# raulmur/ORB_SLAM

Measured on AMD Instinct MI355X. Metric: frames/s ORB extract+match @640x480, 1000 kp, higher is better.
Workload: dtype u8; 1 GPU; vga: 640x480 grayscale stream, 8 levels, nFeatures 1000, S-blocks frames, extract + Hamming top-2 match vs previous frame (BASELINE.json configs[1] + the frame-to-frame match of the metric); resident_frames_per_gpu=2048, lanes=4, parity_checked_frames=0, parity_mismatches=0, library_build_id=b66c8a98a159e636, lane_placement=2

## Files before the change

include/orbx.h:

```cpp
#ifndef ORBX_H
#define ORBX_H

#include <stddef.h>
#include <stdint.h>

#ifdef __cplusplus
extern "C" {
#endif

#define ORBX_OK             0
#define ORBX_EMPTY          1
#define ORBX_ERR_ARG       -1
#define ORBX_ERR_DEVICE    -2
#define ORBX_ERR_CAPACITY  -3
#define ORBX_ERR_GEOMETRY  -4

#define ORBX_HARRIS_SCORE 0
#define ORBX_FAST_SCORE   1

#define ORBX_BLUR_X86_SSE2 0
#define ORBX_BLUR_HALF_UP  1

#define ORBX_FP_ISO          0
#define ORBX_FP_GCC_CONTRACT 1
// ... 109 lines not shown
int orbx_event_destroy(int device, void* event);
int orbx_event_record(void* event, void* stream);
int orbx_stream_wait_event(void* stream, void* event);
int orbx_device_copy_async(void* d_dst, const void* d_src, size_t bytes, void* stream);
int orbx_host_alloc(int device, size_t bytes, void** h_ptr);
int orbx_host_free(int device, void* h_ptr);
int orbx_device_upload_async(void* d_dst, const void* h_src, size_t bytes, void* stream);
int orbx_device_download_async(void* h_dst, const void* d_src, size_t bytes, void* stream);

int orbm_distinctive(const uint8_t* desc, const int32_t* seg_off, int npoints, int32_t* best_idx, int32_t* best_median, int device);
int orbm_distinctive_device(const uint8_t* d_desc, const int32_t* d_seg_off, int npoints, int32_t* d_best_idx,
                            int32_t* d_best_median, void* stream);

#define ORBX_DBG_PLANE      0
#define ORBX_DBG_BLUR       1
#define ORBX_DBG_NMS        2
#define ORBX_DBG_LEVEL_KPS  3
#define ORBX_DBG_BANDS      4
int orbx_debug_set_stop_after(orbx_extractor* h, int stage);
int orbx_debug_set_blur_on_demand(orbx_extractor* h, int mode);
int orbx_debug_stage_timing(orbx_extractor* h, int enable);
int orbx_debug_stage_time(orbx_extractor* h, int stage, double* total_ms, long* launches);
int orbx_debug_level_size(const orbx_extractor* h, int level, int* w, int* hgt);
long orbx_debug_fetch(orbx_extractor* h, int what, int frame, int level, void* host_out, long cap_bytes);
int orbx_debug_geometry(const orbx_params* p, int w, int hgt, int32_t* out, int cap_levels);
int orbx_debug_nth_element(const float* resp, int n, int nth, int32_t* out_perm, int device);
int orbx_debug_eval_math(int kind, const float* in0, const float* in1, float* out0, float* out1, int n, int device);
int orbx_debug_eval_compass(const uint32_t* c, const uint32_t* e, const uint32_t* w, const uint32_t* nn, const uint32_t* ss, uint32_t* out, int n, int t, int device);
int orbx_debug_eval_blur_window(const uint8_t* windows, uint8_t* out, int n, int rounding, int general, int device);

#ifdef __cplusplus
}
#endif
#endif
```

orb_slam_amd/capi.py:

```python
import ctypes
import os
import numpy as np

_HERE = os.path.dirname(os.path.abspath(__file__))
LIB_PATH = os.environ.get("ORBX_LIB") or os.path.join(_HERE, "liborbx.so")

ORBX_OK, ORBX_EMPTY = 0, 1
ORBX_ERR_ARG, ORBX_ERR_DEVICE, ORBX_ERR_CAPACITY, ORBX_ERR_GEOMETRY = -1, -2, -3, -4
HARRIS_SCORE, FAST_SCORE = 0, 1
BLUR_X86_SSE2, BLUR_HALF_UP = 0, 1
DBG_PLANE, DBG_BLUR, DBG_NMS, DBG_LEVEL_KPS, DBG_BANDS = 0, 1, 2, 3, 4
(ST_PYRAMID, ST_FAST_CELLS, ST_QUOTA, ST_CELL_SELECT, ST_LEVEL_SELECT, ST_BLUR, ST_DESCRIBE) = range(7)

KP_DTYPE = np.dtype([("x", "<f4"), ("y", "<f4"), ("size", "<f4"), ("angle", "<f4"),
                     ("response", "<f4"), ("octave", "<i4"), ("class_id", "<i4")])

EXPORTS = [
    "orbx_default_params", "orbx_create", "orbx_destroy", "orbx_get_levels", "orbx_get_scale_factor",
    "orbx_max_keypoints", "orbx_last_error", "orbx_build_id", "orbx_extract", "orbx_extract_batch_device", "orbx_extract_batch_device_phases", "orbx_extract_batch",
    "orbx_to_gray_device", "orbx_extract_color", "orbx_extract_batch_device_color", "orbx_extract_batch_color",
    "orbm_hamming256", "orbm_match_top2", "orbm_match_top2_device", "orbm_match_top2_batch_device", "orbm_match_top2_masked", "orbm_match_top2_masked_device",
    "orbm_count_accepted", "orbm_match_top2_segments", "orbm_match_top2_segments_device", "orbm_distinctive", "orbm_distinctive_device",
    "orbx_device_alloc", "orbx_device_free", "orbx_device_upload", "orbx_device_download",
    "orbx_stream_create", "orbx_stream_create_priority", "orbx_stream_destroy", "orbx_stream_synchronize", "orbx_event_create", "orbx_event_destroy", "orbx_event_record",
    "orbx_stream_wait_event", "orbx_device_copy_async", "orbx_host_alloc", "orbx_host_free", "orbx_device_upload_async", "orbx_device_download_async", "orbx_debug_set_stop_after", "orbx_debug_set_blur_on_demand", "orbx_debug_level_size", "orbx_debug_fetch",
    "orbx_debug_eval_math", "orbx_debug_eval_compass", "orbx_debug_eval_blur_window", "orbx_debug_stage_timing", "orbx_debug_stage_time", "orbx_debug_nth_element", "orbx_debug_geometry",
    "orbm_debug_set_match_path",
    "orbm_debug_get_match_path",
]
EXPORTS_F = [
    "orbf_image_bounds", "orbf_undistort_grid", "orbf_undistort_grid_batch_device", "orbf_features_in_area",
    "orbf_features_in_area_device",
]
EXPORTS_S = ["orbs_lds_bytes", "orbs_debug_set_buckets", "orbs_debug_set_wide_max", "orbs_three_maxima", "orbs_window_search_batch_device", "orbs_list_search_batch_device",
             "orbs_bow_ranges_batch_device", "orbs_triangulation_search_batch_device", "orbs_epipolar_bound", "orbs_agreement_batch_device",
             "orbs_bow_rows_search_batch_device", "orbs_bow_rows_search", "orbs_tri_rows_search_batch_device", "orbs_tri_rows_search"]
PHASE_PYRAMID, PHASE_DETECT, PHASE_DESCRIBE, PHASE_ALL = 1, 2, 4, 7
RULE_MAPPOINTS, RULE_WINDOW, RULE_BEST, RULE_INIT, RULE_BOW, RULE_FREE, RULE_TRIANGULATION = 0, 1, 2, 3, 4, 5, 6
TH_HIGH, TH_LOW = 100, 50
EXPORTS_V = [
    "orbv_create", "orbv_load_text", "orbv_destroy", "orbv_info", "orbv_descend", "orbv_descend_device",
    "orbv_transform", "orbv_transform_batch_device", "orbv_score",
]
EXPORTS_D = ["orbd_create", "orbd_destroy", "orbd_size", "orbd_add", "orbd_add_batch_device", "orbd_erase", "orbd_clear",
             "orbd_query_batch_device", "orbd_query"]
EXPORTS_P = ["orbp_create", "orbp_destroy", "orbp_capacity", "orbp_size", "orbp_clear", "orbp_put", "orbp_put_device", "orbp_erase", "orbp_get",
             "orbp_project_batch_device", "orbp_track_batch_device", "orbp_track", "orbp_project_source_batch_device",
             "orbp_track_source_batch_device", "orbp_track_source", "orbp_refresh_batch_device", "orbp_refresh", "orbp_fuse_batch_device",
# ... 161 lines not shown
        L.orbx_extract_batch_color.argtypes = [vp, vp, vp, ci, ci, ci, ci, ci, vp, vp, vp, ci, vp, vp]
        L.orbm_hamming256.argtypes = [vp, vp]
        L.orbm_match_top2.argtypes = [vp, ci, vp, ci, vp, vp, vp, ci]
        L.orbm_match_top2_device.argtypes = [vp, ci, vp, ci, vp, vp, vp, vp]
        L.orbm_match_top2_batch_device.argtypes = [vp, vp, vp, vp, ci, ci, vp, vp, vp, vp]
        L.orbm_match_top2_masked.argtypes = [vp, ci, vp, ci, vp, vp, vp, vp, ci]
        L.orbm_match_top2_masked_device.argtypes = [vp, ci, vp, ci, vp, vp, vp, vp, vp]
        L.orbm_count_accepted.argtypes = [vp, vp, ci, ci, cf]
        L.orbm_debug_set_match_path.argtypes = [ci]
        L.orbm_debug_get_match_path.argtypes = []
        L.orbs_debug_set_buckets.argtypes = [ci]
        L.orbs_debug_set_wide_max.argtypes = [ci]
        L.orbm_match_top2_segments.argtypes = [vp, ci, vp, ci, vp, vp, vp, vp, vp, ci]
        L.orbm_match_top2_segments_device.argtypes = [vp, ci, vp, ci, vp, vp, vp, vp, vp, vp]
        L.orbx_device_alloc.argtypes = [ci, ctypes.c_size_t, ctypes.POINTER(vp)]
        L.orbx_device_free.argtypes = [ci, vp]
        L.orbx_device_upload.argtypes = [ci, vp, vp, ctypes.c_size_t]
        L.orbx_device_download.argtypes = [ci, vp, vp, ctypes.c_size_t]
        L.orbm_distinctive.argtypes = [vp, vp, ci, vp, vp, ci]
        L.orbm_distinctive_device.argtypes = [vp, vp, ci, vp, vp, vp]
        L.orbx_debug_set_stop_after.argtypes = [vp, ci]
        L.orbx_debug_set_blur_on_demand.argtypes = [vp, ci]
        L.orbx_debug_level_size.argtypes = [vp, ci, ctypes.POINTER(ci), ctypes.POINTER(ci)]
        L.orbx_debug_fetch.argtypes = [vp, ci, ci, ci, vp, cl]
        L.orbx_debug_fetch.restype = cl
        L.orbx_debug_eval_math.argtypes = [ci, vp, vp, vp, vp, ci, ci]
        L.orbx_debug_eval_compass.argtypes = [vp, vp, vp, vp, vp, vp, ci, ci, ci]
        L.orbx_debug_eval_blur_window.argtypes = [vp, vp, ci, ci, ci, ci]
        L.orbx_debug_nth_element.argtypes = [vp, ci, ci, vp, ci]
        L.orbx_debug_geometry.argtypes = [ctypes.POINTER(Params), ci, ci, vp, ci]
        L.orbx_debug_stage_timing.argtypes = [vp, ci]
        L.orbx_debug_stage_time.argtypes = [vp, ci, ctypes.POINTER(ctypes.c_double), ctypes.POINTER(cl)]
        L.orbf_image_bounds.argtypes = [ctypes.POINTER(Camera), ctypes.POINTER(Bounds)]
        L.orbf_undistort_grid.argtypes = [ctypes.POINTER(Camera), ctypes.POINTER(Bounds), vp, ci, vp, vp, vp, ci]
        L.orbf_undistort_grid_batch_device.argtypes = [ctypes.POINTER(Camera), ctypes.POINTER(Bounds), vp, vp, ci, ci, vp, vp, vp, vp]
        L.orbf_features_in_area.argtypes = [ctypes.POINTER(Bounds), vp, ci, vp, vp, vp, vp, ci, vp, vp, ci, ci]
        L.orbf_features_in_area_device.argtypes = [ctypes.POINTER(Bounds), vp, ci, vp, vp, vp, vp, ci, vp, vp, ci, vp, vp]
        L.orbs_lds_bytes.argtypes = [ci, ci]
        L.orbs_lds_bytes.restype = ctypes.c_size_t
        L.orbs_three_maxima.argtypes = [vp, ci, vp]
        L.orbs_three_maxima.restype = None
        L.orbs_window_search_batch_device.argtypes = [ctypes.POINTER(Bounds), ctypes.POINTER(SearchParams), vp, vp, vp, vp, vp, ci, vp,
                                                      vp, vp, vp, vp, vp, vp, ci, ci, vp, vp, vp, vp, vp, vp]
        L.orbs_list_search_batch_device.argtypes = [ctypes.POINTER(SearchParams), vp, vp, vp, vp, vp, ci, vp, vp, vp, vp, vp, vp, vp, ci, ci,
                                                    vp, vp, vp, vp, vp, vp]
        L.orbs_bow_ranges_batch_device.argtypes = [vp, vp, vp, vp, vp, vp, ci, ci, vp, vp, vp]
# ... 291 lines not shown
        if rc != ORBX_OK:
            raise OrbxError(rc, "orbx_debug_set_blur_on_demand")

    STAGE_NAMES = ["pyramid", "fast_cells", "quota", "cell_select", "level_select", "blur", "describe"]

    def stage_timing(self, enable):
        self.L.orbx_debug_stage_timing(self.h, enable)

    def stage_times(self):
        res = {}
        for i, name in enumerate(self.STAGE_NAMES):
            ms, n = ctypes.c_double(), ctypes.c_long()
            self.L.orbx_debug_stage_time(self.h, i, ctypes.byref(ms), ctypes.byref(n))
            res[name] = (ms.value, n.value)
        return res

    def level_size(self, level):
        w, hh = ctypes.c_int(), ctypes.c_int()
        rc = self.L.orbx_debug_level_size(self.h, level, ctypes.byref(w), ctypes.byref(hh))
        if rc != ORBX_OK:
            raise self._err(rc)
        return w.value, hh.value

    def fetch_plane(self, what, level, frame=0):
        w, hh = self.level_size(level)
        out = np.empty((hh, w), dtype=np.uint8)
        rc = self.L.orbx_debug_fetch(self.h, what, frame, level, out.ctypes.data, out.nbytes)
        if rc < 0:
            raise self._err(rc)
        return out

    def fetch_bands(self, level, frame=0):
        out = np.zeros((16384, 8), dtype=np.int32)
        rc = self.L.orbx_debug_fetch(self.h, DBG_BANDS, frame, level, out.ctypes.data, out.nbytes)
        if rc < 0:
            raise self._err(rc)
        return out[:rc // 32].copy()

    def fetch_level_keypoints(self, level, frame=0):
        out = np.zeros((4 * self.max_keypoints + 64, 3), dtype=np.int32)
        rc = self.L.orbx_debug_fetch(self.h, DBG_LEVEL_KPS, frame, level, out.ctypes.data, out.nbytes)
        if rc < 0:
            raise self._err(rc)
        n = rc // 12
        xy = out[:n, :2].copy()
        resp = out[:n, 2].copy().view(np.float32)
# ... 992 lines not shown
```

orb_slam_amd/csrc/k_pyramid.hip:

```cpp
#include <algorithm>
#include <type_traits>

#include "orbx_device.h"
#include "orbx_launch.h"

namespace orbx {


template <bool ALIGNED, bool WINDOW, bool GATHER>
__device__ __forceinline__ void k_resize_body(Batch b, int level) {
    extern __shared__ __attribute__((aligned(16))) uint8_t s_src[];
    const DevGeom& g = b.g;
    const LevelGeom& L = g.lv[level];
    const int RZ_SRC_W = L.rz_pitch;
    const LevelGeom& P = g.lv[level - 1];
    const int tiles_x = (L.w + 255) / 256, tiles_y = (L.h + RZ_ROWS - 1) / RZ_ROWS;
    int frame, tile;
    if (!frame_item(b, blockIdx.x, tiles_x * tiles_y, frame, tile)) return;
    const int tile_y = tile / tiles_x, tile_x = tile - tile_y * tiles_x;
    const int tid = threadIdx.x, lane = tid & 63, wave = wave_id();
    const int bx0 = tile_x * 256, by0 = tile_y * RZ_ROWS;
    const int bx1 = min(bx0 + 255, L.w - 1), by1 = min(by0 + RZ_ROWS - 1, L.h - 1);
    long long sstride;
    const uint8_t* src = plain_plane<GATHER>(b, P, level - 1, frame, sstride);
    const ResizeX* tx = b.tabx + L.tabx_off;
// ... 96 lines not shown
        }
        return;
    }
#pragma unroll
    for (int j = 0; j < RZ_ROWS / 4; j++) {
        const int dy = by0 + wave + 4 * j;
        if (dy >= L.h) break;
        const ResizeY ry = ty[dy];
        const uint8_t* q0 = s_src + (ry.sy0 - r0) * RZ_SRC_W - c0;
        const uint8_t* q1 = s_src + (ry.sy1 - r0) * RZ_SRC_W - c0;
        uint32_t packed = 0;
#pragma unroll
        for (int k = 0; k < 4; k++) {
            const int px = resize_px(q0[rx[k].sx], q0[rx[k].sx1], q1[rx[k].sx], q1[rx[k].sx1], rx[k].a0, rx[k].a1, ry.b0, ry.b1);
            packed |= (uint32_t)(px & 255) << (8 * k);
        }
        *reinterpret_cast<uint32_t*>(dplane + (long long)dy * L.stride + dx0) = packed;
    }
}
template <bool ALIGNED, bool WINDOW>
__global__ __launch_bounds__(256) void k_resize(Batch b, int level) { k_resize_body<ALIGNED, WINDOW, false>(b, level); }
template <bool ALIGNED, bool WINDOW>
__global__ __launch_bounds__(256) void k_resize_gather(Batch b, int level) { k_resize_body<ALIGNED, WINDOW, true>(b, level); }

template <bool ALIGNED, bool GATHER>
__global__ __launch_bounds__(256) void k_pyramid(Batch b, int group) {
    extern __shared__ __attribute__((aligned(16))) uint8_t s_lv[];
    const DevGeom& g = b.g;
    const PyrGroup& pg = g.pyr[group];
    const int frame = blockIdx.z, ix = blockIdx.x, iy = blockIdx.y;
    const int tid = threadIdx.x;
    const int l0 = pg.l0, depth = pg.depth;
    if (group == 0 && ix == 0 && iy == 0 && tid == 0) b.status[frame] = ORBX_OK;
    const int* xt = b.pyr_tab + pg.xtab;
    const int* yt = b.pyr_tab + pg.ytab;
    auto xr = [&](int k, int i, int e) { return xt[(k * (pg.ntx + 1) + i) * 2 + e]; };
    auto yr = [&](int k, int i, int e) { return yt[(k * (pg.nty + 1) + i) * 2 + e]; };
    {
        const LevelGeom& P = g.lv[l0];
        const int xs = xr(0, ix, 0), xe = xr(0, ix, 1), ys = yr(0, iy, 0), ye = yr(0, iy, 1);
        const int nd = ((xe - xs) >> 2) + 1, nr = ye - ys + 1;
        long long sstride;
        const uint8_t* src = plain_plane<GATHER>(b, P, l0, frame, sstride);
        const uint8_t* base = src + (long long)ys * sstride + xs;
        const int xm = P.w - 1 - xs;
        const int total = nr * nd;
// ... 45 lines not shown
            const int X = xs + 4 * G;
            ResizeX rx[4];
#pragma unroll
            for (int j = 0; j < 4; j++) rx[j] = tx[min(X + j, L.w - 1)];
            for (int y = ys + gy; y <= ye; y += ystep) {
                const ResizeY ry = ty[y];
                const uint8_t* q0 = sbuf + (ry.sy0 - sys) * spitch - sxs;
                const uint8_t* q1 = sbuf + (ry.sy1 - sys) * spitch - sxs;
                uint32_t packed = 0;
#pragma unroll
                for (int j = 0; j < 4; j++) {
                    const int px = resize_px(q0[rx[j].sx], q0[rx[j].sx1], q1[rx[j].sx], q1[rx[j].sx1], rx[j].a0, rx[j].a1, ry.b0, ry.b1);
                    packed |= (uint32_t)(px & 255) << (8 * j);
                }
                if (dbuf) *reinterpret_cast<uint32_t*>(dbuf + (y - ys) * dpitch + 4 * G) = packed;
                if (X < own_x1 && y < own_y1) *reinterpret_cast<uint32_t*>(dplane + (long long)y * L.stride + X) = packed;
            }
        }
        __syncthreads();
    }
}


int launch_pyramid(const Batch& b, const HostGeom& hg, hipStream_t stream) {
    const DevGeom& g = hg.g;
    const int F = b.nframes;
    const bool fused_pyramid = g.npyr_groups > 0 && F < PYR_FUSED_MAX_FRAMES;
    const bool al0 = (level0_bits(b) & 3) == 0;
    if (fused_pyramid) {
        for (int gi = 0; gi < g.npyr_groups; gi++) {
            const PyrGroup& pg = g.pyr[gi];
            const bool al = pg.l0 > 0 || al0;
            dim3 grid(pg.ntx, pg.nty, F);
            if (b.img_tab && pg.l0 == 0) {
                if (al) hipLaunchKernelGGL((k_pyramid<true, true>), grid, dim3(256), (size_t)pg.lds_bytes, stream, b, gi);
                else hipLaunchKernelGGL((k_pyramid<false, true>), grid, dim3(256), (size_t)pg.lds_bytes, stream, b, gi);
            } else if (al) hipLaunchKernelGGL((k_pyramid<true, false>), grid, dim3(256), (size_t)pg.lds_bytes, stream, b, gi);
            else hipLaunchKernelGGL((k_pyramid<false, false>), grid, dim3(256), (size_t)pg.lds_bytes, stream, b, gi);
            ORBX_LAUNCH_CHECK();
        }
    } else {
        for (int l = 1; l < g.nlevels; l++) {
            const LevelGeom& L = g.lv[l];
            dim3 grid(frame_item_blocks(b, ((L.w + 255) / 256) * ((L.h + RZ_ROWS - 1) / RZ_ROWS)));
            const bool al = l > 1 || al0;
            const size_t lds = (size_t)L.rz_pitch * L.rz_rows;
            if (b.img_tab && l == 1) {
                if (L.rz_window) {
                    if (al) hipLaunchKernelGGL((k_resize_gather<true, true>), grid, dim3(256), lds, stream, b, l);
                    else hipLaunchKernelGGL((k_resize_gather<false, true>), grid, dim3(256), lds, stream, b, l);
                } else {
                    if (al) hipLaunchKernelGGL((k_resize_gather<true, false>), grid, dim3(256), lds, stream, b, l);
                    else hipLaunchKernelGGL((k_resize_gather<false, false>), grid, dim3(256), lds, stream, b, l);
                }
            } else if (L.rz_window) {
                if (al) hipLaunchKernelGGL((k_resize<true, true>), grid, dim3(256), lds, stream, b, l);
                else hipLaunchKernelGGL((k_resize<false, true>), grid, dim3(256), lds, stream, b, l);
            } else {
                if (al) hipLaunchKernelGGL((k_resize<true, false>), grid, dim3(256), lds, stream, b, l);
                else hipLaunchKernelGGL((k_resize<false, false>), grid, dim3(256), lds, stream, b, l);
            }
            ORBX_LAUNCH_CHECK();
        }
    }
    return ORBX_OK;
}
// ... 3 lines not shown
```

orb_slam_amd/csrc/orbx_api.hip:

```cpp
#include <climits>
#include <cstdio>
#include <cstdlib>
#include <cstring>

#include "orbx_internal.h"

namespace orbx {
int launch_eval_math(int kind, const float* in0, const float* in1, float* out0, float* out1, int n);
int launch_eval_compass(const uint32_t* c, const uint32_t* e, const uint32_t* w, const uint32_t* nn, const uint32_t* ss, uint32_t* out, int n, int t);
int launch_eval_blur_window(const uint8_t* win, uint8_t* out, int n, int ties_even, int general);
void stage_timer_collect(StageTimer& t);
int launch_debug_nth(const float* d_resp, int n, int nth, int* d_out);
int launch_ingest(uint8_t* d_dst, const uint8_t* mapped_src, size_t bytes, hipStream_t stream);
}
using namespace orbx;

struct orbx_extractor {
    orbx_params p;
    std::string err;
    int gw = 0, gh = 0;
    HostGeom hg;
    struct __attribute__((visibility("hidden"))) Geom {
        DevBuf cells, cellrecs, bands, tabx, taby, pyr_tab;
        DevBuf pyr, blur, cand, sel, cstate, csel, cbands, level_total, level_count, status, long_cells;
// ... 135 lines not shown
static int convert(orbx_extractor* h, const uint8_t* src, ptrdiff_t srs, ptrdiff_t sfs, const ImgSrc* tab, unsigned long long tab_bits, int n, int w,
                   int hgt, int fmt, uint8_t* dst, ptrdiff_t drs, ptrdiff_t dfs, uint8_t* dst2, hipStream_t stream);

static int extract_gather(orbx_extractor* h, int fmt, const uint8_t* const* imgs, const ptrdiff_t* row_strides, int nframes, int w, int hgt,
                          orbx_keypoint* d_kps, uint8_t* d_desc, int32_t* d_n, int cap, int32_t* d_status, hipStream_t stream) {
    const int mb = h->p.max_batch;
    size_t gp = 0;
    if (fmt != ORBX_PIX_GRAY8) {
        const int rc = ensure_cring(h, w, hgt, gp);
        if (rc != ORBX_OK) return rc;
    }
    const size_t tab_bytes = (size_t)orbx_extractor::TAB_RING * mb * sizeof(ImgSrc);
    HIPCHK(h, h->d_tab.ensure(tab_bytes));
    HIPCHK(h, h->h_tab.ensure(tab_bytes, hipHostMallocDefault));
    for (Event& e : h->tab_ev) HIPCHK(h, e.ensure());
    for (int f0 = 0; f0 < nframes; f0 += mb) {
        const int n = std::min(mb, nframes - f0);
        const int slot = h->tab_next;
        h->tab_next = (slot + 1) % orbx_extractor::TAB_RING;
        HIPCHK(h, hipEventSynchronize(h->tab_ev[slot]));
        ImgSrc* ht = h->h_tab.as<ImgSrc>() + (size_t)slot * mb;
        ImgSrc* dt = h->d_tab.as<ImgSrc>() + (size_t)slot * mb;
        unsigned long long bits = 0;
        long long min_stride = LLONG_MAX;
        for (int i = 0; i < n; i++) {
            const long long s = row_strides ? (long long)row_strides[f0 + i] : (long long)w * pix_channels(fmt);
            ht[i].data = imgs[f0 + i];
            ht[i].row_stride = s;
            bits |= (uintptr_t)imgs[f0 + i] | (unsigned long long)s;
            min_stride = std::min(min_stride, s);
        }
        HIPCHK(h, hipMemcpyAsync(dt, ht, (size_t)n * sizeof(ImgSrc), hipMemcpyHostToDevice, stream));
        Batch b;
        group_batch(h, b, f0, n, d_kps, d_desc, d_n, cap, d_status);
        if (fmt == ORBX_PIX_GRAY8) {
            b.img_row_stride = min_stride;
            b.img_tab = dt;
            b.img_tab_bits = bits;
            b.img_tab_min_stride = min_stride;
        } else {
            const int rc = convert(h, nullptr, 0, 0, dt, bits, n, w, hgt, fmt, h->d_cring.as(), (ptrdiff_t)gp, (ptrdiff_t)(gp * hgt), nullptr, stream);
            if (rc != ORBX_OK) return rc;
            b.img = h->d_cring.as();
            b.img_row_stride = (long long)gp;
            b.img_frame_stride = (long long)(gp * hgt);
        }
        const int rc = launch_group(h, b, stream);
        if (rc != ORBX_OK) return rc;
        HIPCHK(h, hipEventRecord(h->tab_ev[slot], stream));
        if (fmt == ORBX_PIX_GRAY8) h->last_tab.assign(ht, ht + n);
    }
    return ORBX_OK;
}

static int ensure_cring(orbx_extractor* h, int w, int hgt, size_t& pitch) {
    pitch = ((size_t)w + 15) & ~(size_t)15;
    const size_t bytes = pitch * hgt * h->p.max_batch;
    if (h->d_cring.size() < bytes) {
        HIPCHK(h, hipDeviceSynchronize());
        HIPCHK(h, h->d_cring.ensure(bytes));
    }
    return ORBX_OK;
// ... 428 lines not shown
    if (hipSetDevice(h->p.device) != hipSuccess || hipDeviceSynchronize() != hipSuccess) return ORBX_ERR_DEVICE;
    stage_timer_collect(h->timer);
    h->timer.enabled = enable != 0;
    if (enable == 2) { memset(h->timer.ms, 0, sizeof(h->timer.ms)); memset(h->timer.launches, 0, sizeof(h->timer.launches)); }
    return ORBX_OK;
}

int orbx_debug_stage_time(orbx_extractor* h, int stage, double* total_ms, long* launches) {
    if (!h || stage < 0 || stage >= ST_COUNT) return ORBX_ERR_ARG;
    if (hipSetDevice(h->p.device) != hipSuccess || hipDeviceSynchronize() != hipSuccess) return ORBX_ERR_DEVICE;
    stage_timer_collect(h->timer);
    *total_ms = h->timer.ms[stage];
    *launches = h->timer.launches[stage];
    return ORBX_OK;
}

int orbx_debug_level_size(const orbx_extractor* h, int level, int* w, int* hgt) {
    if (!h || h->gw == 0 || level < 0 || level >= h->hg.g.nlevels) return ORBX_ERR_ARG;
    *w = h->hg.g.lv[level].w;
    *hgt = h->hg.g.lv[level].h;
    return ORBX_OK;
}

long orbx_debug_fetch(orbx_extractor* h, int what, int frame, int level, void* host_out, long cap_bytes) {
    if (!h || !h->have_last || frame < 0 || frame >= h->last.nframes || level < 0 || level >= h->hg.g.nlevels) return ORBX_ERR_ARG;
    if (hipSetDevice(h->p.device) != hipSuccess || hipDeviceSynchronize() != hipSuccess) return ORBX_ERR_DEVICE;
    const DevGeom& g = h->hg.g;
    const LevelGeom& L = g.lv[level];
    const Batch& b = h->last;
    if (what == ORBX_DBG_NMS) {
        const long need = (long)L.w * L.h;
        if (cap_bytes < need) return ORBX_ERR_CAPACITY;
        memset(host_out, 0, need);
        std::vector<CellState> st(g.nbands_total);
        if (hipMemcpy(st.data(), b.cstate + (size_t)frame * g.nbands_total, g.nbands_total * sizeof(CellState), hipMemcpyDeviceToHost) != hipSuccess)
            return ORBX_ERR_DEVICE;
        std::vector<Cand> tmp;
        for (int it = 0; it < g.nbands_total; it++) {
            const BandGeom& bgm = h->hg.bands[it];
            if (bgm.level != level) continue;
            const int n = st[it].n_all;
            if (n <= 0) continue;
            if (n > bgm.cand_cap) return ORBX_ERR_CAPACITY;
            tmp.resize(n);
            if (hipMemcpy(tmp.data(), b.cand + (size_t)frame * g.frame_cands + L.cand_base + bgm.cand_off, (size_t)n * sizeof(Cand), hipMemcpyDeviceToHost) != hipSuccess)
                return ORBX_ERR_DEVICE;
// ... 255 lines not shown
```

orb_slam_amd/csrc/orbx_geometry.hip:

```cpp
#include <cfloat>
#include <climits>
#include <cmath>
#include <cstdlib>
#include <cstring>

#include "orbx_internal.h"

namespace orbx {

static inline int round_even(double v) { return (int)std::lrint(v); }
static inline int floor_int(double v) { int i = (int)v; return i - (i > v); }
static inline int ceil_int(double v) { int i = (int)v; return i + (i < v); }
static inline int16_t sat16(float v) {
    int iv = round_even(v);
    return (int16_t)(iv < SHRT_MIN ? SHRT_MIN : iv > SHRT_MAX ? SHRT_MAX : iv);
}
static inline int align_up(int v, int a) { return (v + a - 1) / a * a; }

static int build_geometry_band(const orbx_params& p, int w, int h, HostGeom& out, std::string& err, const int band_px, const FastShape& shape) {
    const int threads = shape.threads;
    const int nl = p.nlevels;
    if (nl < 1 || nl > MAX_LEVELS) { err = "nlevels out of range [1,16]"; return ORBX_ERR_ARG; }
    if (p.nfeatures < 1) { err = "nfeatures must be >= 1"; return ORBX_ERR_ARG; }
    if (!(p.scale_factor > 1.0f) || p.scale_factor > 2.5f) { err = "scale_factor must be in (1, 2.5]"; return ORBX_ERR_ARG; }
    if (w < 1 || h < 1 || w > 16384 || h > 16384) { err = "image size out of range"; return ORBX_ERR_ARG; }
    if (p.score_type != ORBX_HARRIS_SCORE && p.score_type != ORBX_FAST_SCORE) { err = "score_type"; return ORBX_ERR_ARG; }

    out = HostGeom();
    DevGeom& g = out.g;
    memset(&g, 0, sizeof(g));
    g.nlevels = nl;
    g.score_type = p.score_type;
    g.fp_contract = p.fp_contract ? 1 : 0;
    g.fast_th = std::min(std::max(p.fast_th, 0), 255);
    g.tmin = std::min(g.fast_th, 7);

    const double scaleFactor = (double)p.scale_factor;
    out.scale.assign(nl, 1.f);
    out.inv_scale.assign(nl, 1.f);
    for (int i = 1; i < nl; i++) out.scale[i] = (float)(out.scale[i - 1] * scaleFactor);
// ... 196 lines not shown
                e.sy1 = (int16_t)std::min(std::max(sy + 1, 0), sh - 1);
                e.b0 = sat16((1.f - fy) * 2048);
                e.b1 = sat16(fy * 2048);
                out.taby.push_back(e);
            }
            {
                const ResizeX* tx = out.tabx.data() + L.tabx_off;
                const ResizeY* ty = out.taby.data() + L.taby_off;
                int nd_max = 1, nr_max = 1;
                for (int bx0 = 0; bx0 < dw; bx0 += 256) {
                    const int bx1 = std::min(bx0 + 255, dw - 1);
                    nd_max = std::max(nd_max, ((tx[bx1].sx1 - (tx[bx0].sx & ~3)) >> 2) + 1);
                }
                for (int by0 = 0; by0 < dh; by0 += RZ_ROWS) {
                    const int by1 = std::min(by0 + RZ_ROWS - 1, dh - 1);
                    nr_max = std::max(nr_max, ty[by1].sy1 - ty[by0].sy0 + 1);
                }
                L.rz_pitch = 4 * nd_max + 8;
                L.rz_rows = nr_max;
                int span = 1;
                for (int x0 = 0; x0 < dw; x0 += 4) span = std::max(span, tx[std::min(x0 + 3, dw - 1)].sx1 - tx[x0].sx + 1);
                L.rz_window = span <= 8 ? 1 : 0;
                if (L.rz_pitch * L.rz_rows > 64 * 1024) { err = "resize tile does not fit the LDS"; return ORBX_ERR_CAPACITY; }
            }
        }
    }
    {
        constexpr int tile[2] = {ORBX_PYR_TILE};
        g.npyr_groups = 0;
        out.pyr_tab.clear();
        bool ok = scaleFactor <= 2.0 && nl > 1 && !getenv("ORBX_PYR_PER_LEVEL");
        int l0 = 0;
        while (ok && l0 < nl - 1) {
            if (g.npyr_groups == PYR_MAX_GROUPS) { ok = false; break; }
            PyrGroup pg;
            memset(&pg, 0, sizeof(pg));
            pg.l0 = l0;
            constexpr int depth_cfg[2] = {ORBX_PYR_DEPTH};
            pg.depth = std::min(std::min(l0 == 0 ? depth_cfg[0] : depth_cfg[1], PYR_MAX_DEPTH), nl - 1 - l0);
            const LevelGeom& LD = g.lv[l0 + pg.depth];
            pg.ntx = (LD.w + tile[0] - 1) / tile[0];
            pg.nty = (LD.h + tile[1] - 1) / tile[1];
            auto chain = [&](int n, int tsz, bool is_x, std::vector<int>& tab) {
                const int base = (int)tab.size();
                tab.resize(base + (size_t)(pg.depth + 1) * (n + 1) * 2);
                auto at = [&](int k, int i, int e) -> int& { return tab[base + ((size_t)k * (n + 1) + i) * 2 + e]; };
// ... 130 lines not shown
```

orb_slam_amd/csrc/orbx_internal.h:

```cpp
#pragma once
#include <hip/hip_runtime.h>
#include <stdint.h>
#include <string>
#include <vector>

#include "orbx.h"
#include "orbx_host.h"

namespace orbx {

constexpr int MAX_LEVELS = 16;
constexpr int EDGE = 16;
constexpr int HALF_PATCH = 15;

struct Cand {
    uint32_t pos;
    float resp;
};

struct ResizeX { int16_t sx, sx1, a0, a1; };
struct ResizeY { int16_t sy0, sy1, b0, b1; };

struct LevelGeom {
    int w, h;
    int stride;
    int plane_off;
    int gcols, grows;
    int cellW, cellH;
    int ncells;
    int nfeat_cell;
    int ndesired;
    int cell_base;
    int cand_base;
    int sel_base, sel_cap;
    int slot_base;
    int quad_base;
    int tabx_off, taby_off;
    int rz_window;
    int rz_pitch, rz_rows;
    int btile_base, btiles_x, btiles_y;
    int btile_base_s, btiles_y_s;
    int mb_base, mb_n;
    int mb_strips, mb_bands, mb_band_steps;
    int blur_wvec;
    int blur_sel_last, blur_sel_halo;
    float scale;
    float kp_size;
};

struct CellGeom {
    int16_t x0, y0, x1, y1;
    int32_t skipped;
    int32_t cand_off;
    int32_t cand_cap;
    int32_t band0, nbands;
};

#ifndef ORBX_BLUR_WAVES
#define ORBX_BLUR_WAVES 2
#endif
#ifndef ORBX_BLUR_ON_DEMAND_DEFAULT
#define ORBX_BLUR_ON_DEMAND_DEFAULT 1
// ... 138 lines not shown
    uint8_t* blur;
    Cand* cand;
    Cand* sel;
    CellState* cstate;
    int fallback_hint;
    CellSel* csel;
    CellBands* cbands;
    int32_t* level_total;
    int32_t* level_count;
    int32_t* status;
    int32_t* long_cells;
    orbx_keypoint* out_kps;
    uint8_t* out_desc;
    int32_t* out_n;
    int32_t* out_status;
    int cap;
    int nframes;
    int xcd_affinity;
    int od_min_frames;
    int blur_on_demand;
    const ImgSrc* img_tab;
    unsigned long long img_tab_bits;
    long long img_tab_min_stride;
};

static inline unsigned long long level0_bits(const Batch& b) {
    return b.img_tab ? b.img_tab_bits : ((uintptr_t)b.img | (unsigned long long)b.img_row_stride | (unsigned long long)b.img_frame_stride);
}
static inline long long level0_min_stride(const Batch& b) { return b.img_tab ? b.img_tab_min_stride : b.img_row_stride; }

struct ColorArgs {
    const uint8_t* src;
    long long src_row_stride, src_frame_stride;
    const ImgSrc* tab;
    unsigned long long tab_bits;
    uint8_t* dst;
    uint8_t* dst2;
    long long dst_row_stride, dst_frame_stride;
    int w, h;
    int f0;
    int cpr, items;
};
static inline int pix_channels(int fmt) {
    switch (fmt) {
        case ORBX_PIX_GRAY8: return 1;
        case ORBX_PIX_RGB8: case ORBX_PIX_BGR8: return 3;
        case ORBX_PIX_RGBA8: case ORBX_PIX_BGRA8: return 4;
        default: return 0;
    }
}
int launch_to_gray(const ColorArgs& a, int nframes, int fmt, hipStream_t stream);

struct HostGeom {
    DevGeom g;
    std::vector<CellGeom> cells;
    std::vector<CellRec> cellrecs;
    std::vector<BandGeom> bands;
    std::vector<ResizeX> tabx;
    std::vector<ResizeY> taby;
    std::vector<int> pyr_tab;
    std::vector<int> features_per_level;
    std::vector<float> scale, inv_scale;
};

int build_geometry(const orbx_params& p, int w, int h, HostGeom& out, std::string& err);

enum Stage { ST_PYRAMID = 0, ST_FAST_CELLS, ST_QUOTA, ST_CELL_SELECT, ST_LEVEL_SELECT, ST_BLUR, ST_DESCRIBE, ST_COUNT };

struct StageTimer {
    bool enabled = false;
    std::vector<hipEvent_t> pool;
    std::vector<int> pool_stage;
    double ms[ST_COUNT] = {0};
    long launches[ST_COUNT] = {0};
};

struct SideStream {
    Stream aux;
    Event fork, join;
};
int launch_extract(const Batch& b, const HostGeom& hg, hipStream_t stream, int stop_after, StageTimer* timer, const SideStream* side,
                   int phases = ORBX_PHASE_ALL);
bool describe_od_supported(const Batch& b, const HostGeom& hg);
int launch_describe_od(const Batch& b, const HostGeom& hg, hipStream_t stream);

}
```

Before: 481,700 frames/s.

## Add strip-based pyramid resize kernel staging source rows in LDS via async loads

```diff
diff --git a/include/orbx.h b/include/orbx.h
--- a/include/orbx.h
+++ b/include/orbx.h
@@ -155,6 +155,7 @@
 int orbx_debug_stage_timing(orbx_extractor* h, int enable);
 int orbx_debug_stage_time(orbx_extractor* h, int stage, double* total_ms, long* launches);
 int orbx_debug_level_size(const orbx_extractor* h, int level, int* w, int* hgt);
+int orbx_debug_resize_form(const orbx_extractor* h, int level, int* form, int* rows_out);
 long orbx_debug_fetch(orbx_extractor* h, int what, int frame, int level, void* host_out, long cap_bytes);
 int orbx_debug_geometry(const orbx_params* p, int w, int hgt, int32_t* out, int cap_levels);
 int orbx_debug_nth_element(const float* resp, int n, int nth, int32_t* out_perm, int device);
diff --git a/orb_slam_amd/capi.py b/orb_slam_amd/capi.py
--- a/orb_slam_amd/capi.py
+++ b/orb_slam_amd/capi.py
@@ -23,7 +23,7 @@
     "orbm_count_accepted", "orbm_match_top2_segments", "orbm_match_top2_segments_device", "orbm_distinctive", "orbm_distinctive_device",
     "orbx_device_alloc", "orbx_device_free", "orbx_device_upload", "orbx_device_download",
     "orbx_stream_create", "orbx_stream_create_priority", "orbx_stream_destroy", "orbx_stream_synchronize", "orbx_event_create", "orbx_event_destroy", "orbx_event_record",
-    "orbx_stream_wait_event", "orbx_device_copy_async", "orbx_host_alloc", "orbx_host_free", "orbx_device_upload_async", "orbx_device_download_async", "orbx_debug_set_stop_after", "orbx_debug_set_blur_on_demand", "orbx_debug_level_size", "orbx_debug_fetch",
+    "orbx_stream_wait_event", "orbx_device_copy_async", "orbx_host_alloc", "orbx_host_free", "orbx_device_upload_async", "orbx_device_download_async", "orbx_debug_set_stop_after", "orbx_debug_set_blur_on_demand", "orbx_debug_level_size", "orbx_debug_resize_form", "orbx_debug_fetch",
     "orbx_debug_eval_math", "orbx_debug_eval_compass", "orbx_debug_eval_blur_window", "orbx_debug_stage_timing", "orbx_debug_stage_time", "orbx_debug_nth_element", "orbx_debug_geometry",
     "orbm_debug_set_match_path",
     "orbm_debug_get_match_path",
@@ -231,6 +231,8 @@
         L.orbx_debug_set_stop_after.argtypes = [vp, ci]
         L.orbx_debug_set_blur_on_demand.argtypes = [vp, ci]
         L.orbx_debug_level_size.argtypes = [vp, ci, ctypes.POINTER(ci), ctypes.POINTER(ci)]
+        if hasattr(L, "orbx_debug_resize_form"):
+            L.orbx_debug_resize_form.argtypes = [vp, ci, ctypes.POINTER(ci), ctypes.POINTER(ci)]
         L.orbx_debug_fetch.argtypes = [vp, ci, ci, ci, vp, cl]
         L.orbx_debug_fetch.restype = cl
         L.orbx_debug_eval_math.argtypes = [ci, vp, vp, vp, vp, ci, ci]
@@ -568,6 +570,13 @@
             raise self._err(rc)
         return w.value, hh.value
 
+    def resize_form(self, level):
+        form, rows = ctypes.c_int(), ctypes.c_int()
+        rc = self.L.orbx_debug_resize_form(self.h, level, ctypes.byref(form), ctypes.byref(rows))
+        if rc != ORBX_OK:
+            raise OrbxError(rc, "orbx_debug_resize_form")
+        return form.value, rows.value
+
     def fetch_plane(self, what, level, frame=0):
         w, hh = self.level_size(level)
         out = np.empty((hh, w), dtype=np.uint8)
diff --git a/orb_slam_amd/csrc/k_pyramid.hip b/orb_slam_amd/csrc/k_pyramid.hip
--- a/orb_slam_amd/csrc/k_pyramid.hip
+++ b/orb_slam_amd/csrc/k_pyramid.hip
@@ -1,6 +1,7 @@
 #include <algorithm>
 #include <type_traits>
 
+#include "k_resize_strip.h"
 #include "orbx_device.h"
 #include "orbx_launch.h"
 
@@ -143,6 +144,135 @@
 __global__ __launch_bounds__(256) void k_resize(Batch b, int level) { k_resize_body<ALIGNED, WINDOW, false>(b, level); }
 template <bool ALIGNED, bool WINDOW>
 __global__ __launch_bounds__(256) void k_resize_gather(Batch b, int level) { k_resize_body<ALIGNED, WINDOW, true>(b, level); }
+
+struct RzsCols {
+    uint32_t sel[4], apair[4];
+    int wa, sh;
+};
+__device__ __forceinline__ void rzs_load_cols(const ResizeX* tx, int w, int dcol, RzsCols& c) {
+    ResizeX rx[4];
+#pragma unroll
+    for (int k = 0; k < 4; k++) rx[k] = tx[min(4 * dcol + k, w - 1)];
+    const int w0 = rx[0].sx;
+    c.wa = w0 & ~3;
+    c.sh = w0 & 3;
+#pragma unroll
+    for (int k = 0; k < 4; k++) {
+        c.sel[k] = (uint32_t)(rx[k].sx - w0) | 0x0C000C00u | ((uint32_t)(rx[k].sx1 - w0) << 16);
+        c.apair[k] = (uint32_t)(uint16_t)rx[k].a0 | ((uint32_t)(uint16_t)rx[k].a1 << 16);
+    }
+}
+__device__ __forceinline__ void rzs_hrow(const uint8_t* s_src, int off, const RzsCols& c, uint32_t (&d)[4]) {
+    const uint32_t* p = reinterpret_cast<const uint32_t*>(s_src + off);
+    const uint32_t d0 = p[0], d1 = p[1], d2 = p[2];
+    const uint32_t lo = __builtin_amdgcn_alignbyte(d1, d0, (uint32_t)c.sh), hi = __builtin_amdgcn_alignbyte(d2, d1, (uint32_t)c.sh);
+#pragma unroll
+    for (int k = 0; k < 4; k++) d[k] = __builtin_amdgcn_udot2(as_us2v(__builtin_amdgcn_perm(hi, lo, c.sel[k])), as_us2v(c.apair[k]), 0u, false) >> 4;
+}
+__device__ __forceinline__ uint32_t rzs_vpack(const uint32_t (&da)[4], const uint32_t (&db)[4], uint32_t b0s, uint32_t b1s) {
+    uint32_t packed = 0;
+#pragma unroll
+    for (int k = 0; k < 4; k++) packed |= ((__umulhi(da[k], b0s) + __umulhi(db[k], b1s) + 2u) >> 2) << (8 * k);
+    return packed;
+}
+
+template <bool GATHER, int NG>
+__device__ __forceinline__ void k_resize_strip_body(Batch b, int level, int rows_out, int nstrips, unsigned magic) {
+    extern __shared__ __attribute__((aligned(16))) uint8_t s_src[];
+    const DevGeom& g = b.g;
+    const LevelGeom& L = g.lv[level];
+    const LevelGeom& P = g.lv[level - 1];
+    int frame, strip;
+    if (!frame_item_magic(b, blockIdx.x, (unsigned)nstrips, magic, frame, strip)) return;
+    const int tid = threadIdx.x, lane = tid & 63, wave = wave_id();
+    long long sstride64;
+    const uint8_t* src = plain_plane<GATHER>(b, P, level - 1, frame, sstride64);
+    const int sstride = (int)sstride64;
+    const ResizeX* tx = b.tabx + L.tabx_off;
+    const ResizeY* ty = b.taby + L.taby_off;
+    const int RPW = rows_out >> 2;
+    const int row0 = strip * rows_out + wave * RPW;
+    const uint2 ryl = *reinterpret_cast<const uint2*>(ty + min(row0 + min(lane, RPW - 1), L.h - 1));
+    const int ngroups = NG ? NG : rzs_groups(L.w);
+    const int rem = rzs_rem_cols(L.w);
+    const bool rowpar = rem <= RZS_ROWPAR_MAX;
+    const int shift = rzs_rowpar_shift(rem);
+    auto group_col = [&](int gi) { return gi == ngroups - 1 && rowpar ? 64 * gi + rzs_rowpar_slot(lane, shift) : rzs_loop_col(gi, lane); };
+    RzsCols cols[NG ? NG : 1];
+    if (NG) {
+#pragma unroll
+        for (int gi = 0; gi < NG; gi++) rzs_load_cols(tx, L.w, group_col(gi), cols[gi]);
+    }
+    __builtin_amdgcn_sched_barrier(0);
+    const StripSpan sp = rzs_span(ty, L.h, rows_out, strip, sstride64, rzs_readable(level == 1, sstride64, P.w));
+    const int r0 = sp.r0, nchunks = (int)sp.chunks;
+    {
+        typedef const void __attribute__((address_space(1))) * gptr_t;
+        typedef void __attribute__((address_space(3))) * lptr_t;
+        const uint8_t* base = src + (long long)r0 * sstride64;
+        if (tid < sp.tail_dwords)
+            *reinterpret_cast<uint32_t*>(s_src + 16 * nchunks + 4 * tid) = *reinterpret_cast<const uint32_t*>(base + 16 * (long long)nchunks + 4 * tid);
+        for (int q0 = 64 * wave; q0 < nchunks; q0 += 256)
+            if (q0 + lane < nchunks) __builtin_amdgcn_global_load_lds((gptr_t)(base + 16 * (q0 + lane)), (lptr_t)(s_src + 16 * q0), 16, 0, 0);
+        asm volatile("s_waitcnt vmcnt(0)" ::: "memory");
+    }
+    __syncthreads();
+    uint8_t* dplane = b.pyr + (long long)frame * g.frame_plane_bytes + L.plane_off;
+    const unsigned dstride = (unsigned)L.stride;
+    const int nrows = min(RPW, L.h - row0);
+    auto process = [&](int gi, const RzsCols& c) {
+        const int dcol = group_col(gi);
+        if (gi == ngroups - 1 && rowpar) {
+            const int slot = rzs_rowpar_slot(lane, shift);
+            for (int pass = 0; pass * (64 >> shift) < RPW; pass++) {
+                const int j = rzs_rowpar_row(lane, shift, pass);
+                const uint32_t ry_rows = (uint32_t)__shfl((int)ryl.x, min(j, RPW - 1)), ry_w = (uint32_t)__shfl((int)ryl.y, min(j, RPW - 1));
+                const int dy = row0 + j;
+                if (slot < rem && j < RPW && dy < L.h) {
+                    const int sy0 = (int16_t)(ry_rows & 0xffffu), sy1 = (int16_t)(ry_rows >> 16);
+                    uint32_t da[4], db[4];
+                    rzs_hrow(s_src, (sy0 - r0) * sstride + c.wa, c, da);
+                    rzs_hrow(s_src, (sy1 - r0) * sstride + c.wa, c, db);
+                    *reinterpret_cast<uint32_t*>(dplane + ((unsigned)dy * dstride + 4u * (unsigned)dcol)) = rzs_vpack(da, db, ry_w << 16, ry_w & 0xffff0000u);
+                }
+            }
+        } else if (4 * dcol < L.w) {
+            int have = -1;
+            uint32_t cur[4] = {0, 0, 0, 0};
+            for (int j = 0; j < nrows; j++) {
+                const int dy = row0 + j;
+                const uint32_t ry_rows = (uint32_t)__builtin_amdgcn_readlane((int)ryl.x, j), ry_w = (uint32_t)__builtin_amdgcn_readlane((int)ryl.y, j);
+                const int sy0 = (int16_t)(ry_rows & 0xffffu), sy1 = (int16_t)(ry_rows >> 16);
+                const uint32_t b0s = ry_w << 16, b1s = ry_w & 0xffff0000u;
+                if (sy0 != have) rzs_hrow(s_src, (sy0 - r0) * sstride + c.wa, c, cur);
+                uint32_t t[4];
+#pragma unroll
+                for (int k = 0; k < 4; k++) t[k] = __umulhi(cur[k], b0s);
+                asm volatile("" : "+v"(t[0]), "+v"(t[1]), "+v"(t[2]), "+v"(t[3]));
+                if (sy1 != sy0) rzs_hrow(s_src, (sy1 - r0) * sstride + c.wa, c, cur);
+                have = sy1;
+                uint32_t packed = 0;
+#pragma unroll
+                for (int k = 0; k < 4; k++) packed |= ((t[k] + __umulhi(cur[k], b1s) + 2u) >> 2) << (8 * k);
+                *reinterpret_cast<uint32_t*>(dplane + ((unsigned)dy * dstride + 4u * (unsigned)dcol)) = packed;
+            }
+        }
+    };
+    if constexpr (NG != 0) {
+#pragma unroll
+        for (int gi = 0; gi < NG; gi++) process(gi, cols[gi]);
+    } else {
+        for (int gi = 0; gi < ngroups; gi++) {
+            rzs_load_cols(tx, L.w, group_col(gi), cols[0]);
+            process(gi, cols[0]);
+        }
+    }
+}
+typedef void (*resize_strip_fn)(Batch, int, int, int, unsigned);
+template <int NG>
+__global__ __launch_bounds__(256) void k_resize(Batch b, int level, int rows_out, int nstrips, unsigned magic) { k_resize_strip_body<false, NG>(b, level, rows_out, nstrips, magic); }
+template <int NG>
+__global__ __launch_bounds__(256) void k_resize_gather(Batch b, int level, int rows_out, int nstrips, unsigned magic) { k_resize_strip_body<true, NG>(b, level, rows_out, nstrips, magic); }
 
 template <bool ALIGNED, bool GATHER>
 __global__ __launch_bounds__(256) void k_pyramid(Batch b, int group) {
@@ -234,6 +364,27 @@
 }
 
 
+int resize_form(const Batch& b, const HostGeom& hg, int level, StripChoice& sc) {
+    const DevGeom& g = hg.g;
+    sc = StripChoice{0, 0};
+    if (level < 1 || level >= g.nlevels) return RZ_FORM_TILED;
+    if (g.npyr_groups > 0 && b.nframes < PYR_FUSED_MAX_FRAMES) return RZ_FORM_FUSED;
+    const LevelGeom& L = g.lv[level];
+    if (level >= 2 || (level0_max_stride(b) == g.lv[0].w && (level0_bits(b) & 3) == 0)) sc = StripChoice{L.rs_rows, L.rs_lds};
+    else sc = resize_strip_choice(hg, level, level0_max_stride(b), level0_bits(b));
+    return sc.rows_out ? RZ_FORM_STRIP : RZ_FORM_TILED;
+}
+
+template <int NG>
+static void launch_resize_strip(const Batch& b, int l, const StripChoice& sc, hipStream_t stream) {
+    const LevelGeom& L = b.g.lv[l];
+    const int nstrips = rzs_strips(L.h, sc.rows_out);
+    const unsigned magic = frame_item_magic_of(nstrips);
+    dim3 grid(frame_item_blocks(b, nstrips));
+    const resize_strip_fn fn = b.img_tab && l == 1 ? static_cast<resize_strip_fn>(&k_resize_gather<NG>) : static_cast<resize_strip_fn>(&k_resize<NG>);
+    hipLaunchKernelGGL(fn, grid, dim3(256), (size_t)sc.lds_bytes, stream, b, l, sc.rows_out, nstrips, magic);
+}
+
 int launch_pyramid(const Batch& b, const HostGeom& hg, hipStream_t stream) {
     const DevGeom& g = hg.g;
     const int F = b.nframes;
@@ -254,6 +405,18 @@
     } else {
         for (int l = 1; l < g.nlevels; l++) {
             const LevelGeom& L = g.lv[l];
+            StripChoice sc;
+            if (resize_form(b, hg, l, sc) == RZ_FORM_STRIP) {
+                switch (rzs_groups(L.w)) {
+                    case 1: launch_resize_strip<1>(b, l, sc, stream); break;
+                    case 2: launch_resize_strip<2>(b, l, sc, stream); break;
+                    case 3: launch_resize_strip<3>(b, l, sc, stream); break;
+                    case 4: launch_resize_strip<4>(b, l, sc, stream); break;
+                    default: launch_resize_strip<0>(b, l, sc, stream); break;
+                }
+                ORBX_LAUNCH_CHECK();
+                continue;
+            }
             dim3 grid(frame_item_blocks(b, ((L.w + 255) / 256) * ((L.h + RZ_ROWS - 1) / RZ_ROWS)));
             const bool al = l > 1 || al0;
             const size_t lds = (size_t)L.rz_pitch * L.rz_rows;
diff --git a/orb_slam_amd/csrc/k_resize_strip.h b/orb_slam_amd/csrc/k_resize_strip.h
--- /dev/null
+++ b/orb_slam_amd/csrc/k_resize_strip.h
@@ -0,0 +1,78 @@
+#pragma once
+#include <stdint.h>
+
+#include "orb_math.h"
+
+namespace orbx {
+
+constexpr int RZS_WG_PER_CU = 8;
+constexpr int RZS_LDS_BUDGET = 160 * 1024 / RZS_WG_PER_CU;
+constexpr int RZS_ROWS_MIN = 12, RZS_ROWS_CAP = 48;
+constexpr int RZS_SLACK = 16;
+constexpr int RZS_ROWPAR_MAX = 32;
+
+enum { RZ_FORM_TILED = 0, RZ_FORM_STRIP = 1, RZ_FORM_FUSED = 2 };
+
+ORBX_HD long long rzs_readable(bool src_is_level0, long long stride, int src_w) {
+    if (!src_is_level0) return stride;
+    const long long w16 = (long long)((src_w + 15) & ~15);
+    return stride < w16 ? stride : w16;
+}
+
+struct StripSpan {
+    int by0, by1;
+    int r0, r1;
+    long long bytes;
+    long long chunks;
+    int tail_dwords;
+    long long lds_bytes;
+};
+
+template <class RY>
+ORBX_HD StripSpan rzs_span(const RY* ty, int h, int rows_out, int strip, long long stride, long long readable) {
+    StripSpan s;
+    s.by0 = strip * rows_out;
+    s.by1 = imin(s.by0 + rows_out - 1, h - 1);
+    s.r0 = ty[s.by0].sy0;
+    s.r1 = ty[s.by1].sy1;
+    s.bytes = (long long)(s.r1 - s.r0) * stride + readable;
+    s.chunks = s.bytes >> 4;
+    s.tail_dwords = (int)(s.bytes & 15) >> 2;
+    s.lds_bytes = ((s.bytes + 15) & ~15ll) + RZS_SLACK;
+    return s;
+}
+
+ORBX_HD int rzs_strips(int h, int rows_out) { return (h + rows_out - 1) / rows_out; }
+
+template <class RY>
+inline long long rzs_lds_bytes(const RY* ty, int h, int rows_out, long long stride, long long readable) {
+    long long m = 0;
+    for (int s = 0; s < rzs_strips(h, rows_out); s++) {
+        const long long v = rzs_span(ty, h, rows_out, s, stride, readable).lds_bytes;
+        m = v > m ? v : m;
+    }
+    return m;
+}
+
+template <class RY>
+inline int rzs_pick_rows(const RY* ty, int h, long long stride, long long readable, int budget = RZS_LDS_BUDGET, int cap = RZS_ROWS_CAP) {
+    for (int r = cap & ~3; r >= RZS_ROWS_MIN; r -= 4)
+        if (rzs_lds_bytes(ty, h, r, stride, readable) <= (long long)budget) return r;
+    return 0;
+}
+
+ORBX_HD int rzs_dword_cols(int w) { return (w + 3) >> 2; }
+ORBX_HD int rzs_groups(int w) { return (rzs_dword_cols(w) + 63) >> 6; }
+ORBX_HD int rzs_rem_cols(int w) { return rzs_dword_cols(w) - 64 * (rzs_groups(w) - 1); }
+ORBX_HD bool rzs_rowpar(int w) { return rzs_rem_cols(w) <= RZS_ROWPAR_MAX; }
+ORBX_HD int rzs_rowpar_shift(int rem) {
+    int s = 0;
+    while ((1 << s) < rem) s++;
+    return s;
+}
+ORBX_HD int rzs_loop_col(int g, int lane) { return 64 * g + lane; }
+ORBX_HD int rzs_rowpar_slot(int lane, int shift) { return lane & ((1 << shift) - 1); }
+ORBX_HD int rzs_rowpar_row(int lane, int shift, int pass) { return pass * (64 >> shift) + (lane >> shift); }
+ORBX_HD long long rzs_window_off(int sy, int r0, long long stride, int sx0) { return (long long)(sy - r0) * stride + (sx0 & ~3); }
+
+}
diff --git a/orb_slam_amd/csrc/orbx_api.hip b/orb_slam_amd/csrc/orbx_api.hip
--- a/orb_slam_amd/csrc/orbx_api.hip
+++ b/orb_slam_amd/csrc/orbx_api.hip
@@ -181,13 +181,14 @@
         ImgSrc* ht = h->h_tab.as<ImgSrc>() + (size_t)slot * mb;
         ImgSrc* dt = h->d_tab.as<ImgSrc>() + (size_t)slot * mb;
         unsigned long long bits = 0;
-        long long min_stride = LLONG_MAX;
+        long long min_stride = LLONG_MAX, max_stride = 0;
         for (int i = 0; i < n; i++) {
             const long long s = row_strides ? (long long)row_strides[f0 + i] : (long long)w * pix_channels(fmt);
             ht[i].data = imgs[f0 + i];
             ht[i].row_stride = s;
             bits |= (uintptr_t)imgs[f0 + i] | (unsigned long long)s;
             min_stride = std::min(min_stride, s);
+            max_stride = std::max(max_stride, s);
         }
         HIPCHK(h, hipMemcpyAsync(dt, ht, (size_t)n * sizeof(ImgSrc), hipMemcpyHostToDevice, stream));
         Batch b;
@@ -197,6 +198,7 @@
             b.img_tab = dt;
             b.img_tab_bits = bits;
             b.img_tab_min_stride = min_stride;
+            b.img_tab_max_stride = max_stride;
         } else {
             const int rc = convert(h, nullptr, 0, 0, dt, bits, n, w, hgt, fmt, h->d_cring.as(), (ptrdiff_t)gp, (ptrdiff_t)(gp * hgt), nullptr, stream);
             if (rc != ORBX_OK) return rc;
@@ -671,6 +673,14 @@
     return ORBX_OK;
 }
 
+int orbx_debug_resize_form(const orbx_extractor* h, int level, int* form, int* rows_out) {
+    if (!h || !h->have_last || !form || !rows_out || level < 1 || level >= h->hg.g.nlevels) return ORBX_ERR_ARG;
+    StripChoice sc;
+    *form = resize_form(h->last, h->hg, level, sc);
+    *rows_out = sc.rows_out;
+    return ORBX_OK;
+}
+
 long orbx_debug_fetch(orbx_extractor* h, int what, int frame, int level, void* host_out, long cap_bytes) {
     if (!h || !h->have_last || frame < 0 || frame >= h->last.nframes || level < 0 || level >= h->hg.g.nlevels) return ORBX_ERR_ARG;
     if (hipSetDevice(h->p.device) != hipSuccess || hipDeviceSynchronize() != hipSuccess) return ORBX_ERR_DEVICE;
diff --git a/orb_slam_amd/csrc/orbx_geometry.hip b/orb_slam_amd/csrc/orbx_geometry.hip
--- a/orb_slam_amd/csrc/orbx_geometry.hip
+++ b/orb_slam_amd/csrc/orbx_geometry.hip
@@ -4,6 +4,7 @@
 #include <cstdlib>
 #include <cstring>
 
+#include "k_resize_strip.h"
 #include "orbx_internal.h"
 
 namespace orbx {
@@ -16,6 +17,26 @@
     return (int16_t)(iv < SHRT_MIN ? SHRT_MIN : iv > SHRT_MAX ? SHRT_MAX : iv);
 }
 static inline int align_up(int v, int a) { return (v + a - 1) / a * a; }
+
+StripChoice resize_strip_choice(const HostGeom& hg, int level, long long src_stride, unsigned long long src_bits) {
+    StripChoice sc = {0, 0};
+    const DevGeom& g = hg.g;
+    if (level < 1 || level >= g.nlevels) return sc;
+    const LevelGeom& L = g.lv[level];
+    const LevelGeom& P = g.lv[level - 1];
+    if (!L.rz_window) return sc;
+    long long stride = P.stride;
+    if (level == 1) {
+        stride = src_stride;
+        if (((src_bits | (unsigned long long)stride) & 3) != 0 || stride < P.w) return sc;
+    }
+    const long long readable = rzs_readable(level == 1, stride, P.w);
+    if (stride > RZS_LDS_BUDGET) return sc;
+    const ResizeY* ty = hg.taby.data() + L.taby_off;
+    sc.rows_out = rzs_pick_rows(ty, L.h, stride, readable);
+    if (sc.rows_out) sc.lds_bytes = (int)rzs_lds_bytes(ty, L.h, sc.rows_out, stride, readable);
+    return sc;
+}
 
 static int build_geometry_band(const orbx_params& p, int w, int h, HostGeom& out, std::string& err, const int band_px, const FastShape& shape) {
     const int threads = shape.threads;
@@ -258,6 +279,9 @@
                 for (int x0 = 0; x0 < dw; x0 += 4) span = std::max(span, tx[std::min(x0 + 3, dw - 1)].sx1 - tx[x0].sx + 1);
                 L.rz_window = span <= 8 ? 1 : 0;
                 if (L.rz_pitch * L.rz_rows > 64 * 1024) { err = "resize tile does not fit the LDS"; return ORBX_ERR_CAPACITY; }
+                const StripChoice sc = resize_strip_choice(out, l, l == 1 ? (long long)sw : 0, 0);
+                L.rs_rows = sc.rows_out;
+                L.rs_lds = sc.lds_bytes;
             }
         }
     }
diff --git a/orb_slam_amd/csrc/orbx_internal.h b/orb_slam_amd/csrc/orbx_internal.h
--- a/orb_slam_amd/csrc/orbx_internal.h
+++ b/orb_slam_amd/csrc/orbx_internal.h
@@ -38,6 +38,7 @@
     int tabx_off, taby_off;
     int rz_window;
     int rz_pitch, rz_rows;
+    int rs_rows, rs_lds;
     int btile_base, btiles_x, btiles_y;
     int btile_base_s, btiles_y_s;
     int mb_base, mb_n;
@@ -222,12 +223,14 @@
     const ImgSrc* img_tab;
     unsigned long long img_tab_bits;
     long long img_tab_min_stride;
+    long long img_tab_max_stride;
 };
 
 static inline unsigned long long level0_bits(const Batch& b) {
     return b.img_tab ? b.img_tab_bits : ((uintptr_t)b.img | (unsigned long long)b.img_row_stride | (unsigned long long)b.img_frame_stride);
 }
 static inline long long level0_min_stride(const Batch& b) { return b.img_tab ? b.img_tab_min_stride : b.img_row_stride; }
+static inline long long level0_max_stride(const Batch& b) { return b.img_tab ? b.img_tab_max_stride : b.img_row_stride; }
 
 struct ColorArgs {
     const uint8_t* src;
@@ -265,6 +268,10 @@
 
 int build_geometry(const orbx_params& p, int w, int h, HostGeom& out, std::string& err);
 
+struct StripChoice { int rows_out, lds_bytes; };
+StripChoice resize_strip_choice(const HostGeom& hg, int level, long long src_stride, unsigned long long src_bits);
+int resize_form(const Batch& b, const HostGeom& hg, int level, StripChoice& sc);
+
 enum Stage { ST_PYRAMID = 0, ST_FAST_CELLS, ST_QUOTA, ST_CELL_SELECT, ST_LEVEL_SELECT, ST_BLUR, ST_DESCRIBE, ST_COUNT };
 
 struct StageTimer {
```

New measurement: 498,100 frames/s, median of 6. 3.4% higher.
